# bdaiinstitute/vlfm

Measured on NVIDIA H100. Metric: value-map steps/sec (ITM+cone-fuse), higher is better.
Workload: dtype f16

## Files before the change

### vlfm_b200/csrc/gemm_wgmma.cu

```cuda
#include <cuda.h>
#include <cuda_fp16.h>
#include <math.h>
#include <stdlib.h>

#include "common.cuh"

namespace vlfm {

constexpr int BM = 128;
constexpr int BK = 64;
constexpr int GEMM_THREADS = 384;
constexpr int GEMM_CONSUMERS = 256;

__device__ __forceinline__ void mbar_expect_tx(uint32_t bar, uint32_t bytes) {
  asm volatile("mbarrier.arrive.expect_tx.shared::cta.b64 _, [%0], %1;" ::"r"(bar), "r"(bytes) : "memory");
}
__device__ __forceinline__ void mbar_arrive(uint32_t bar) {
  asm volatile("mbarrier.arrive.shared::cta.b64 _, [%0];" ::"r"(bar) : "memory");
}
__device__ __forceinline__ void tma_load_2d(uint32_t dst, const CUtensorMap* map, int x, int y, uint32_t bar) {
  asm volatile(
      "cp.async.bulk.tensor.2d.shared::cluster.global.mbarrier::complete_tx::bytes [%0], [%1, {%3, %4}], [%2];"
      ::"r"(dst), "l"(map), "r"(bar), "r"(x), "r"(y) : "memory");
}
__device__ __forceinline__ uint64_t wgmma_desc_k128(uint32_t saddr) {
  return (uint64_t)((saddr & 0x3FFFF) >> 4) | ((uint64_t)1 << 16) | ((uint64_t)(1024 >> 4) << 32) | ((uint64_t)1 << 62);
}
__device__ __forceinline__ void wg_fence() { asm volatile("wgmma.fence.sync.aligned;" ::: "memory"); }
__device__ __forceinline__ void wg_commit() { asm volatile("wgmma.commit_group.sync.aligned;" ::: "memory"); }
template <int PENDING>
__device__ __forceinline__ void wg_wait() { asm volatile("wgmma.wait_group.sync.aligned %0;" ::"n"(PENDING) : "memory"); }

#define VLFM_D4(d, i) "+f"(d[i]), "+f"(d[i + 1]), "+f"(d[i + 2]), "+f"(d[i + 3])
#define VLFM_D16(d, i) VLFM_D4(d, i), VLFM_D4(d, i + 4), VLFM_D4(d, i + 8), VLFM_D4(d, i + 12)
template <int BN> struct Wgmma;
template <> struct Wgmma<32> {
  static __device__ __forceinline__ void mma(float (&d)[16], uint64_t a, uint64_t b, uint32_t acc) {
    asm volatile(
        "{\n\t.reg .pred p;\n\tsetp.ne.b32 p, %18, 0;\n\t"
        "wgmma.mma_async.sync.aligned.m64n32k16.f32.f16.f16 "
        "{%0,%1,%2,%3,%4,%5,%6,%7,%8,%9,%10,%11,%12,%13,%14,%15}, %16, %17, p, 1, 1, 0, 0;\n\t}"
        : VLFM_D16(d, 0) : "l"(a), "l"(b), "r"(acc));
  }
};
template <> struct Wgmma<64> {
  static __device__ __forceinline__ void mma(float (&d)[32], uint64_t a, uint64_t b, uint32_t acc) {
    asm volatile(
        "{\n\t.reg .pred p;\n\tsetp.ne.b32 p, %34, 0;\n\t"
        "wgmma.mma_async.sync.aligned.m64n64k16.f32.f16.f16 "
        "{%0,%1,%2,%3,%4,%5,%6,%7,%8,%9,%10,%11,%12,%13,%14,%15,"
        "%16,%17,%18,%19,%20,%21,%22,%23,%24,%25,%26,%27,%28,%29,%30,%31}, %32, %33, p, 1, 1, 0, 0;\n\t}"
        : VLFM_D16(d, 0), VLFM_D16(d, 16) : "l"(a), "l"(b), "r"(acc));
  }
};
template <> struct Wgmma<96> {
  static __device__ __forceinline__ void mma(float (&d)[48], uint64_t a, uint64_t b, uint32_t acc) {
    asm volatile(
        "{\n\t.reg .pred p;\n\tsetp.ne.b32 p, %50, 0;\n\t"
        "wgmma.mma_async.sync.aligned.m64n96k16.f32.f16.f16 "
        "{%0,%1,%2,%3,%4,%5,%6,%7,%8,%9,%10,%11,%12,%13,%14,%15,"
        "%16,%17,%18,%19,%20,%21,%22,%23,%24,%25,%26,%27,%28,%29,%30,%31,"
        "%32,%33,%34,%35,%36,%37,%38,%39,%40,%41,%42,%43,%44,%45,%46,%47}, %48, %49, p, 1, 1, 0, 0;\n\t}"
        : VLFM_D16(d, 0), VLFM_D16(d, 16), VLFM_D16(d, 32) : "l"(a), "l"(b), "r"(acc));
  }
};
template <> struct Wgmma<128> {
  static __device__ __forceinline__ void mma(float (&d)[64], uint64_t a, uint64_t b, uint32_t acc) {
    asm volatile(
        "{\n\t.reg .pred p;\n\tsetp.ne.b32 p, %66, 0;\n\t"
        "wgmma.mma_async.sync.aligned.m64n128k16.f32.f16.f16 "
        "{%0,%1,%2,%3,%4,%5,%6,%7,%8,%9,%10,%11,%12,%13,%14,%15,"
        "%16,%17,%18,%19,%20,%21,%22,%23,%24,%25,%26,%27,%28,%29,%30,%31,"
        "%32,%33,%34,%35,%36,%37,%38,%39,%40,%41,%42,%43,%44,%45,%46,%47,"
        "%48,%49,%50,%51,%52,%53,%54,%55,%56,%57,%58,%59,%60,%61,%62,%63}, %64, %65, p, 1, 1, 0, 0;\n\t}"
        : VLFM_D16(d, 0), VLFM_D16(d, 16), VLFM_D16(d, 32), VLFM_D16(d, 48) : "l"(a), "l"(b), "r"(acc));
  }
};
#undef VLFM_D16
#undef VLFM_D4

struct GemmArgs {
  const float* bias;
  void* out;
  int M, N, K, ldo, epi;
  int kb_per_split;
  long long split_stride;
// ... 375 lines not shown
      const uint32_t a0 = smem_u32(sA + s * A_BYTES) + (uint32_t)wg * (64 * BK * 2), b0 = smem_u32(sB + s * B_BYTES);
      wg_fence();
#pragma unroll
      for (int k = 0; k < BK / 16; ++k)
        Wgmma<BN>::mma(acc, wgmma_desc_k128(a0 + k * 32), wgmma_desc_k128(b0 + k * 32), (kb > kb_lo || k > 0) ? 1u : 0u);
      wg_commit();
      if (f < BN) {
        const uint8_t* wrow = sB + (size_t)s * B_BYTES + (size_t)f * 128;
        const int k0 = (kb - kb_lo) * BK + hk * 32;
        float a[GEMM_TAIL_MAX];
#pragma unroll
        for (int r = 0; r < GEMM_TAIL_MAX; ++r) a[r] = 0.f;
#pragma unroll
        for (int c = 0; c < 4; ++c) {
          const uint4 wv = *reinterpret_cast<const uint4*>(wrow + (((hk * 4 + c) ^ (f & 7)) << 4));
          const __half2* wh = reinterpret_cast<const __half2*>(&wv);
#pragma unroll
          for (int r = 0; r < GEMM_TAIL_MAX; ++r) {
            if (r < g.tail_rows) {
              const uint4 xv = *reinterpret_cast<const uint4*>(sx + (size_t)r * kslice + k0 + c * 8);
              const __half2* xh = reinterpret_cast<const __half2*>(&xv);
#pragma unroll
              for (int e = 0; e < 4; ++e) {
                const float2 xf = __half22float2(xh[e]), wf = __half22float2(wh[e]);
                a[r] = fmaf(xf.x, wf.x, a[r]); a[r] = fmaf(xf.y, wf.y, a[r]);
              }
            }
          }
        }
#pragma unroll
        for (int r = 0; r < GEMM_TAIL_MAX; ++r) tacc[r] += a[r];
      }
      wg_wait<1>();
      if (kb > kb_lo) {
        __syncwarp();
        if (lane == 0) mbar_arrive(empty0 + 8 * (s == 0 ? STAGES - 1 : s - 1));
      }
      if (++s == STAGES) { s = 0; ph ^= 1; }
    }
    wg_wait<0>();
#pragma unroll
    for (int r = 0; r < GEMM_TAIL_MAX; ++r) tacc[r] += __shfl_xor_sync(0xffffffffu, tacc[r], 1);
    if (s_cl == 1) {
      if (hk == 0 && f < BN && n_blk * BN + f < g.N) {
#pragma unroll
        for (int r = 0; r < GEMM_TAIL_MAX; ++r)
          if (r < g.tail_rows) epilogue_store2(g, CS_BM + r, n_blk * BN + f, tacc[r] + sbias[f], 0.f, false, false);
      }
      epilogue_frag<BN>(acc, wg * 64 + wq * 16, n_blk, g, false, true, sbias);
    } else {
      asm volatile("bar.sync 1, 512;" ::: "memory");
      const int r_up = wg * 64 + wq * 16 + (lane >> 2), cq = (lane & 3) * 2;
#pragma unroll
      for (int j = 0; j < BN / 8; ++j) {
        *reinterpret_cast<float2*>(part + r_up * LDP + j * 8 + cq) = make_float2(acc[4 * j], acc[4 * j + 1]);
        *reinterpret_cast<float2*>(part + (r_up + 8) * LDP + j * 8 + cq) = make_float2(acc[4 * j + 2], acc[4 * j + 3]);
      }
      if (hk == 0 && f < BN) {
#pragma unroll
        for (int r = 0; r < GEMM_TAIL_MAX; ++r)
          if (r < g.tail_rows) part[(CS_BM + r) * LDP + f] = tacc[r];
      }
    }
  }
  if (s_cl > 1) {
    cluster_sync_all();
    if (warp >= 4) {
      const int et = threadIdx.x - (CS_THREADS - CS_CONSUMERS);
      const int rows = CS_BM + g.tail_rows, r0 = rank * rows / s_cl, r1 = (rank + 1) * rows / s_cl;
      const uint32_t base = smem_u32(part);
      for (int i = et; i < (r1 - r0) * (BN / 2); i += CS_CONSUMERS) {
        const int row = r0 + i / (BN / 2), c = (i % (BN / 2)) * 2, n = n_blk * BN + c;
        if (n >= g.N) continue;
        const uint32_t off = base + (uint32_t)(row * LDP + c) * 4;
        float2 sum = ld_peer_f2(off, 0);
        for (int p = 1; p < s_cl; ++p) { const float2 v = ld_peer_f2(off, p); sum.x += v.x; sum.y += v.y; }
        epilogue_store2(g, row, n, sum.x + sbias[c], sum.y + sbias[c + 1], n + 1 < g.N, false);
      }
    }
    cluster_sync_all();
  }
}

template <int BN, int STAGES>
__global__ void __launch_bounds__(GEMM_THREADS, 1)
gemm_f16x2_wgmma_kernel(const __grid_constant__ CUtensorMap tmA, const __grid_constant__ CUtensorMap tmAl,
                        const __grid_constant__ CUtensorMap tmB, const __grid_constant__ CUtensorMap tmBl, GemmArgs g) {
  constexpr uint32_t A_BYTES = BM * BK * 2, B_BYTES = BN * BK * 2;

  extern __shared__ uint8_t smem_raw[];
  uint8_t* sA = smem_align_1024(smem_raw);
  uint8_t* sAl = sA + STAGES * A_BYTES;
  uint8_t* sB = sAl + STAGES * A_BYTES;
  uint8_t* sBl = sB + STAGES * B_BYTES;
  uint64_t* bars = reinterpret_cast<uint64_t*>(sBl + STAGES * B_BYTES);
  const uint32_t full0 = smem_u32(bars), empty0 = smem_u32(bars + STAGES);
  float* sbias = reinterpret_cast<float*>(bars + 2 * STAGES);

  pdl_trigger();
  const int warp = threadIdx.x >> 5, lane = threadIdx.x & 31;
  const int n_blk = blockIdx.x, m_blk = blockIdx.y;
  const int kb_begin = blockIdx.z * g.kb_per_split;
  const int num_k = min((g.K + BK - 1) / BK - kb_begin, g.kb_per_split);
  const bool split = gridDim.z > 1;

  if (warp == 0 && lane == 0) {
    asm volatile("prefetch.tensormap [%0];" ::"l"(&tmA) : "memory");
    asm volatile("prefetch.tensormap [%0];" ::"l"(&tmAl) : "memory");
    asm volatile("prefetch.tensormap [%0];" ::"l"(&tmB) : "memory");
    asm volatile("prefetch.tensormap [%0];" ::"l"(&tmBl) : "memory");
    for (int i = 0; i < STAGES; ++i) { mbar_init(full0 + 8 * i, 1); mbar_init(empty0 + 8 * i, GEMM_CONSUMERS / 32); }
    asm volatile("fence.mbarrier_init.release.cluster;" ::: "memory");
    asm volatile("fence.proxy.async.shared::cta;" ::: "memory");
  }
  __syncthreads();

  if (warp == 0) {
    if (lane == 0) {
      const int pre = num_k < STAGES ? num_k : STAGES;
      const uint32_t a_tx = (uint32_t)g.a_box_rows * BK * 2;
      for (int kb = 0; kb < pre; ++kb) {
        mbar_expect_tx(full0 + 8 * kb, 2 * (a_tx + B_BYTES));
        tma_load_2d(smem_u32(sB + kb * B_BYTES), &tmB, (kb_begin + kb) * BK, n_blk * BN, full0 + 8 * kb);
        tma_load_2d(smem_u32(sBl + kb * B_BYTES), &tmBl, (kb_begin + kb) * BK, n_blk * BN, full0 + 8 * kb);
      }
      pdl_wait();
      for (int kb = 0; kb < pre; ++kb) {
        tma_load_2d(smem_u32(sA + kb * A_BYTES), &tmA, (kb_begin + kb) * BK, m_blk * BM, full0 + 8 * kb);
        tma_load_2d(smem_u32(sAl + kb * A_BYTES), &tmAl, (kb_begin + kb) * BK, m_blk * BM, full0 + 8 * kb);
      }
      int s = pre == STAGES ? 0 : pre; uint32_t ph = pre == STAGES ? 1 : 0;
      for (int kb = pre; kb < num_k; ++kb) {
        mbar_wait(empty0 + 8 * s, ph ^ 1);
        mbar_expect_tx(full0 + 8 * s, 2 * (a_tx + B_BYTES));
        tma_load_2d(smem_u32(sA + s * A_BYTES), &tmA, (kb_begin + kb) * BK, m_blk * BM, full0 + 8 * s);
        tma_load_2d(smem_u32(sAl + s * A_BYTES), &tmAl, (kb_begin + kb) * BK, m_blk * BM, full0 + 8 * s);
        tma_load_2d(smem_u32(sB + s * B_BYTES), &tmB, (kb_begin + kb) * BK, n_blk * BN, full0 + 8 * s);
        tma_load_2d(smem_u32(sBl + s * B_BYTES), &tmBl, (kb_begin + kb) * BK, n_blk * BN, full0 + 8 * s);
        if (++s == STAGES) { s = 0; ph ^= 1; }
      }
    }
  } else if (warp >= 4) {
    const int wg = (warp >> 2) - 1, wq = warp & 3;
    const int et = threadIdx.x - (GEMM_THREADS - GEMM_CONSUMERS);
    const int wg_row0 = m_blk * BM + wg * 64;
    const bool active = wg_row0 < g.M;
    if (et < BN) { const int n = n_blk * BN + et; sbias[et] = (g.bias && n < g.N) ? __ldg(g.bias + n) : 0.f; }
    asm volatile("bar.sync 1, 256;" ::: "memory");
    pdl_wait();
    if (!active) {
      int s = 0; uint32_t ph = 0;
      for (int kb = 0; kb < num_k; ++kb) {
        mbar_wait(full0 + 8 * s, ph);
        __syncwarp();
        if (lane == 0) mbar_arrive(empty0 + 8 * s);
        if (++s == STAGES) { s = 0; ph ^= 1; }
      }
      return;
    }
    float acc[BN / 2], corr[BN / 2];
#pragma unroll
    for (int i = 0; i < BN / 2; ++i) { acc[i] = 0.f; corr[i] = 0.f; }
    int s = 0; uint32_t ph = 0;
    for (int kb = 0; kb < num_k; ++kb) {
      mbar_wait(full0 + 8 * s, ph);
      const uint32_t wg_off = (uint32_t)wg * (64 * BK * 2);
      const uint32_t a0 = smem_u32(sA + s * A_BYTES) + wg_off, al0 = smem_u32(sAl + s * A_BYTES) + wg_off;
      const uint32_t b0 = smem_u32(sB + s * B_BYTES), bl0 = smem_u32(sBl + s * B_BYTES);
      wg_fence();
#pragma unroll
      for (int k = 0; k < BK / 16; ++k) {
        const uint64_t da = wgmma_desc_k128(a0 + k * 32), dal = wgmma_desc_k128(al0 + k * 32);
        const uint64_t db = wgmma_desc_k128(b0 + k * 32), dbl = wgmma_desc_k128(bl0 + k * 32);
        const uint32_t first = (kb > 0 || k > 0) ? 1u : 0u;
        Wgmma<BN>::mma(acc, da, db, first);
        Wgmma<BN>::mma(corr, dal, db, first);
        Wgmma<BN>::mma(corr, da, dbl, 1u);
      }
      wg_commit();
      wg_wait<1>();
      if (kb > 0) {
        __syncwarp();
        if (lane == 0) mbar_arrive(empty0 + 8 * (s == 0 ? STAGES - 1 : s - 1));
      }
      if (++s == STAGES) { s = 0; ph ^= 1; }
    }
    wg_wait<0>();
#pragma unroll
    for (int i = 0; i < BN / 2; ++i) acc[i] = fmaf(corr[i], 1.f / X2_SCALE, acc[i]);
    epilogue_frag<BN>(acc, wg_row0 + wq * 16, n_blk, g, split, blockIdx.z == 0, sbias);
  }
}

typedef CUresult (*EncodeTiledFn)(CUtensorMap*, CUtensorMapDataType, cuuint32_t, void*, const cuuint64_t*,
                                  const cuuint64_t*, const cuuint32_t*, const cuuint32_t*, CUtensorMapInterleave,
                                  CUtensorMapSwizzle, CUtensorMapL2promotion, CUtensorMapFloatOOBfill);

static EncodeTiledFn get_encode() {
  static EncodeTiledFn fn = nullptr;
  static bool tried = false;
  if (!tried) {
    tried = true;
    void* p = nullptr;
    cudaDriverEntryPointQueryResult q;
    if (cudaGetDriverEntryPoint("cuTensorMapEncodeTiled", &p, cudaEnableDefault, &q) == cudaSuccess &&
        q == cudaDriverEntryPointSuccess)
      fn = reinterpret_cast<EncodeTiledFn>(p);
  }
  return fn;
}

static int make_map(CUtensorMap* m, const void* base, int rows, int cols, int ld, int boxRows) {
  EncodeTiledFn enc = get_encode();
  if (!enc) { set_error("cuTensorMapEncodeTiled entry point unavailable"); return VLFM_E_DRIVER; }
  cuuint64_t dims[2] = {(cuuint64_t)cols, (cuuint64_t)rows};
  cuuint64_t strides[1] = {(cuuint64_t)ld * 2};
  cuuint32_t box[2] = {(cuuint32_t)BK, (cuuint32_t)boxRows};
  cuuint32_t estr[2] = {1, 1};
  CUresult r = enc(m, CU_TENSOR_MAP_DATA_TYPE_FLOAT16, 2, const_cast<void*>(base), dims, strides, box, estr,
                   CU_TENSOR_MAP_INTERLEAVE_NONE, CU_TENSOR_MAP_SWIZZLE_128B, CU_TENSOR_MAP_L2_PROMOTION_L2_256B,
                   CU_TENSOR_MAP_FLOAT_OOB_FILL_NONE);
  if (r != CUDA_SUCCESS) { set_error("cuTensorMapEncodeTiled failed (%d) rows=%d cols=%d ld=%d", (int)r, rows, cols, ld); return VLFM_E_DRIVER; }
  return VLFM_OK;
}

template <int BN, int STAGES, bool SILU = false>
static int launch_gemm(const CUtensorMap& ta, const void* W, int ldw, const GemmArgs& g, cudaStream_t st) {
  if constexpr (!SILU) {
    if (g.epi == VLFM_EPI_BIAS_SILU_F16) return launch_gemm<BN, STAGES, true>(ta, W, ldw, g, st);
  }
  CUtensorMap tb;
  int rc = make_map(&tb, W, g.N, g.K, ldw, BN);
  if (rc) return rc;
  constexpr size_t smem = (size_t)STAGES * (BM * BK * 2 + BN * BK * 2) + 2 * STAGES * 8 + 1024 + BN * 4 +
                          (size_t)GEMM_TAIL_MAX * GEMM_TAIL_KMAX * 2;
  static_assert(smem <= 227 * 1024, "GEMM stage ring exceeds the 227 KB a block may use");
  static bool configured = false;
  if (!configured) {
    rc = check_cuda(cudaFuncSetAttribute(gemm_f16_wgmma_kernel<BN, STAGES, SILU>, cudaFuncAttributeMaxDynamicSharedMemorySize, (int)smem), "cudaFuncSetAttribute(gemm)");
    if (rc) return rc;
    configured = true;
  }
  const int num_k = (g.K + BK - 1) / BK;
  dim3 grid((g.N + BN - 1) / BN, g.tail_rows > 0 ? g.M / BM : (g.M + BM - 1) / BM, (num_k + g.kb_per_split - 1) / g.kb_per_split);
  if (g.sk.ctas > 0) grid = dim3(g.sk.ctas);
  rc = check_cuda(launch_pdl(gemm_f16_wgmma_kernel<BN, STAGES, SILU>, grid, dim3(GEMM_THREADS), smem, st, ta, tb, g), "gemm_f16_wgmma_kernel");
  if (rc) return rc;
  count_launch();
  return VLFM_OK;
}


template <int BN, int STAGES>
static int launch_gemm_x2(const CUtensorMap& ta, const CUtensorMap& tal, const void* W, const void* Wl, int ldw, const GemmArgs& g, cudaStream_t st) {
  CUtensorMap tb, tbl;
  int rc = make_map(&tb, W, g.N, g.K, ldw, BN);
  if (!rc) rc = make_map(&tbl, Wl, g.N, g.K, ldw, BN);
  if (rc) return rc;
  constexpr size_t smem = (size_t)STAGES * 2 * (BM * BK * 2 + BN * BK * 2) + 2 * STAGES * 8 + 1024 + BN * 4;
  static_assert(smem <= 227 * 1024, "x2 GEMM stage ring exceeds the 227 KB a block may use");
  static bool configured = false;
  if (!configured) {
    rc = check_cuda(cudaFuncSetAttribute(gemm_f16x2_wgmma_kernel<BN, STAGES>, cudaFuncAttributeMaxDynamicSharedMemorySize, (int)smem), "cudaFuncSetAttribute(gemm x2)");
    if (rc) return rc;
    configured = true;
  }
  const int num_k = (g.K + BK - 1) / BK;
  dim3 grid((g.N + BN - 1) / BN, (g.M + BM - 1) / BM, (num_k + g.kb_per_split - 1) / g.kb_per_split);
  rc = check_cuda(launch_pdl(gemm_f16x2_wgmma_kernel<BN, STAGES>, grid, dim3(GEMM_THREADS), smem, st, ta, tal, tb, tbl, g), "gemm_f16x2_wgmma_kernel");
  if (rc) return rc;
  count_launch();
  return VLFM_OK;
}

template <int BN, int STAGES>
struct Csplit {
  static constexpr size_t smem = (size_t)STAGES * (CS_BM * BK * 2 + BN * BK * 2) + 2 * STAGES * 8 + 1024 + BN * 4 +
                                 (size_t)GEMM_TAIL_MAX * GEMM_TAIL_KMAX * 2;
  static_assert(smem <= 227 * 1024, "cluster-split GEMM stage ring exceeds the 227 KB a block may use");
  static int configure() {
    static int rc = -1;
    if (rc < 0) rc = check_cuda(cudaFuncSetAttribute(gemm_f16_csplit_wgmma_kernel<BN, STAGES>, cudaFuncAttributeMaxDynamicSharedMemorySize, (int)smem),
                                "cudaFuncSetAttribute(gemm csplit)");
    return rc;
  }
  static int max_clusters(int s) {
    static int fit[9] = {-1, -1, -1, -1, -1, -1, -1, -1, -1};
    if (fit[s] < 0) {
      fit[s] = 0;
      if (configure()) return 0;
      cudaLaunchConfig_t cfg{};
      cfg.gridDim = dim3(s); cfg.blockDim = dim3(CS_THREADS); cfg.dynamicSmemBytes = smem;
      cudaLaunchAttribute attr[1];
      attr[0].id = cudaLaunchAttributeClusterDimension;
      attr[0].val.clusterDim.x = s; attr[0].val.clusterDim.y = 1; attr[0].val.clusterDim.z = 1;
      cfg.attrs = attr; cfg.numAttrs = 1;
      int n = 0;
      if (cudaOccupancyMaxActiveClusters(&n, gemm_f16_csplit_wgmma_kernel<BN, STAGES>, &cfg) == cudaSuccess) fit[s] = n;
      else cudaGetLastError();
    }
    return fit[s];
  }
  static int launch(const CUtensorMap& ta, const void* W, int ldw, const GemmArgs& g, int s, cudaStream_t st) {
    CUtensorMap tb;
    int rc = make_map(&tb, W, g.N, g.K, ldw, BN);
    if (!rc) rc = configure();
    if (rc) return rc;
    cudaLaunchConfig_t cfg{};
    cfg.gridDim = dim3(((g.N + BN - 1) / BN) * s); cfg.blockDim = dim3(CS_THREADS); cfg.dynamicSmemBytes = smem; cfg.stream = st;
    cudaLaunchAttribute attr[2];
    attr[0].id = cudaLaunchAttributeClusterDimension;
    attr[0].val.clusterDim.x = s; attr[0].val.clusterDim.y = 1; attr[0].val.clusterDim.z = 1;
    attr[1].id = cudaLaunchAttributeProgrammaticStreamSerialization;
    attr[1].val.programmaticStreamSerializationAllowed = 1;
    cfg.attrs = attr; cfg.numAttrs = pdl_enabled() ? 2 : 1;
    rc = check_cuda(cudaLaunchKernelEx(&cfg, gemm_f16_csplit_wgmma_kernel<BN, STAGES>, ta, tb, g), "gemm_f16_csplit_wgmma_kernel");
    if (rc) return rc;
    count_launch();
    return VLFM_OK;
  }
};

}

using namespace vlfm;

static int gemm_dispatch(const void* d_A, const void* d_W, int M, int N, int K, int lda, int ldw, GemmArgs g, void* stream, float* d_partials,
                         size_t partial_bytes, SplitK* layout, bool csplit);

static int sm_count() {
  static int sms = 0;
  if (!sms) { int dev = 0; cudaGetDevice(&dev); if (cudaDeviceGetAttribute(&sms, cudaDevAttrMultiProcessorCount, dev) != cudaSuccess || sms < 1) sms = 132; }
  return sms;
}

extern "C" int vlfm_gemm_f16(const void* d_A, const void* d_W, const float* d_bias, void* d_out, int M, int N,
                             int K, int lda, int ldw, int ldo, int epilogue, void* stream) {
  if (!d_A || !d_W || !d_out || M < 1 || N < 1 || K < 1) { set_error("vlfm_gemm_f16: bad argument"); return VLFM_E_INVALID; }
  if ((K & 7) || (lda & 7) || (ldw & 7) || (ldo & 7) || ((uintptr_t)d_A & 15) || ((uintptr_t)d_W & 15) || ((uintptr_t)d_out & 15)) {
    set_error("vlfm_gemm_f16: K, lda, ldw, ldo must be multiples of 8 and pointers 16-byte aligned"); return VLFM_E_INVALID; }
  const bool csplit = (epilogue & VLFM_EPI_CLUSTER_SPLIT) != 0 && (epilogue & ~VLFM_EPI_CLUSTER_SPLIT) != VLFM_EPI_BIAS_SILU_F16;
  epilogue &= ~VLFM_EPI_CLUSTER_SPLIT;
  if (epilogue < 0 || (epilogue > 4 && epilogue != VLFM_EPI_BIAS_SILU_F16)) { set_error("vlfm_gemm_f16: unknown epilogue %d", epilogue); return VLFM_E_INVALID; }
  GemmArgs g{d_bias, d_out, M, N, K, ldo, epilogue, (K + BK - 1) / BK, 0, nullptr, 0, 0, 0, nullptr, BM};
  return gemm_dispatch(d_A, d_W, M, N, K, lda, ldw, g, stream, nullptr, 0, nullptr, csplit);
}

constexpr double CS_RED_FIXED_BYTES = 16384;
constexpr long long CS_MIN_WEIGHTS = 8ll << 20;
static bool csplit_eligible(int M, int N, int K) {
  const char* e = getenv("VLFM_GEMM_CSPLIT");
  const int mode = (e && e[0]) ? atoi(e) : 1;
// ... 84 lines not shown
      return launch_gemm<128, 6>(ta, d_W, ldw, g, st);
    }
  }
  if (tiles128 <= sms && !resid) {
    const int bns[4] = {128, 96, 64, 32};
    long long best = -1;
    for (int bn : bns) {
      const long long tl = (long long)rt * ((N + bn - 1) / bn), cols = (tl + sms - 1) / sms * bn;
      if (best < 0 || cols < best) { best = cols; best_bn = bn; }
    }
  } else {
    double best_t = 1e30;
    const int bns[3] = {128, 64, 32};
    for (int tm = 0; tm < (tail ? 2 : 1); ++tm) {
      const bool use_tail = tail && tm == 0;
      const int mte = use_tail ? M / BM : mt;
      for (int bi = 0; bi < 3; ++bi) {
        const int bn = bns[bi], nt = (N + bn - 1) / bn;
        int smax = resid && !(d_partials && tiles128 < sms) ? num_k / 4 : 1;
        if (smax < 1) smax = 1;
        if (smax > 8) smax = 8;
        if (smax > split_cap) smax = (int)split_cap;
        for (int sp = 1; sp <= smax; ++sp) {
          const double ctas = (double)mte * nt * sp;
          const int kb = (num_k + sp - 1) / sp;
          const double waves = (double)(long)((ctas + sms - 1) / sms);
          const double active = ctas < sms ? ctas : sms;
          const double kb_kbytes = (double)(128 + bn) * 128 / 1024.0;
          double per_kb = active * kb_kbytes / 5500.0;
          if (per_kb < 0.33) per_kb = 0.33;
          double c0 = bn == 128 ? 3.8 + 0.22 * sp : (bn == 64 ? 3.0 : 2.6) + (sp > 1 ? 0.1 * sp : 0.0);
          if (use_tail) c0 += bn == 128 ? 0.9 : 0.3;
          const double t = waves * (c0 + kb * per_kb);
          if (t < best_t) { best_t = t; best_bn = bn; best_s = sp; best_tail = use_tail; }
        }
      }
    }
  }
  if (force) {
    int fb = 0, fs = 0;
    if (sscanf(force, "%d:%d", &fb, &fs) == 2 && (fb == 128 || fb == 96 || fb == 64 || fb == 32) && fs >= 1) {
      best_bn = fb;
      best_s = resid ? (fs > num_k ? num_k : fs) : 1;
      if (best_s > split_cap) best_s = (int)split_cap;
    }
  }
  g.kb_per_split = (num_k + best_s - 1) / best_s;
  if (best_tail) { g.a_tail = (const __half*)d_A + (size_t)(M / BM) * BM * lda; g.lda = lda; g.tail_rows = rem; g.tail_row0 = (M / BM) * BM; }
  const int launched_splits = (num_k + g.kb_per_split - 1) / g.kb_per_split;
  if (d_partials && launched_splits > 1 && resid && (size_t)launched_splits * (size_t)M * (size_t)N * 4 <= partial_bytes) {
    g.epi = VLFM_EPI_PARTIAL_F32; g.out = d_partials; g.ldo = N; g.split_stride = (long long)M * N;
    if (layout) *layout = SplitK{launched_splits, (long long)M * N};
  }
  if (best_bn == 128) return launch_gemm<128, 6>(ta, d_W, ldw, g, st);
  if (best_bn == 96) return launch_gemm<96, 7>(ta, d_W, ldw, g, st);
  if (best_bn == 64) return launch_gemm<64, 8>(ta, d_W, ldw, g, st);
  return launch_gemm<32, 8>(ta, d_W, ldw, g, st);
}

extern "C" int vlfm_layernorm(const float* d_x, const float* d_gamma, const float* d_beta, void* d_out16, float* d_out32,
                   int rows, int D, int ldx, int ldo16, int ldo32, float eps, void* stream);
namespace vlfm {
int layernorm_reduce_impl(float* d_x, const float* d_partials, const SplitK& sk, const float* d_gamma, const float* d_beta, void* d_out16,
                          void* d_out16_lo, float* d_out32, int rows, int D, int ldx, int ldo16, int ldo32, float eps, void* stream);
}

extern "C" int vlfm_gemm_f16_resid_ln(const void* d_A, const void* d_W, const float* d_bias, float* d_x, int M, int N, int K,
                                      int lda, int ldw, int ldx, const float* d_gamma, const float* d_beta, void* d_out16,
                                      int ld16, float* d_out32, int ld32, float eps, float* d_partials, size_t partial_bytes, void* stream) {
  if (!d_A || !d_W || !d_x || !d_gamma || !d_beta || (!d_out16 && !d_out32) || M < 1 || N < 1 || K < 1) {
    set_error("vlfm_gemm_f16_resid_ln: bad argument"); return VLFM_E_INVALID; }
  if ((K & 7) || (lda & 7) || (ldw & 7) || (ldx & 7) || (N & 3) || (ld16 & 3) || (ld32 & 3) || ((uintptr_t)d_A & 15) || ((uintptr_t)d_W & 15) ||
      ((uintptr_t)d_x & 15) || ((uintptr_t)d_partials & 15)) { set_error("vlfm_gemm_f16_resid_ln: alignment (K, strides %% 8; N %% 4; 16-byte pointers)"); return VLFM_E_INVALID; }
  int rc = layernorm_check("vlfm_gemm_f16_resid_ln", d_x, d_gamma, d_beta, d_out16, nullptr, d_out32, N, ldx, ld16, ld32);
  if (rc) return rc;
  GemmArgs g{d_bias, d_x, M, N, K, ldx, VLFM_EPI_BIAS_RESID_F32, (K + BK - 1) / BK, 0, nullptr, 0, 0, 0, nullptr, BM};
  SplitK layout;
  rc = gemm_dispatch(d_A, d_W, M, N, K, lda, ldw, g, stream, d_partials, partial_bytes, &layout, d_partials != nullptr);
  if (rc) return rc;
  if (layout.splits != 1) return layernorm_reduce_impl(d_x, d_partials, layout, d_gamma, d_beta, d_out16, nullptr, d_out32, M, N, ldx, ld16, ld32, eps, stream);
  return vlfm_layernorm(d_x, d_gamma, d_beta, d_out16, d_out32, M, N, ldx, ld16, ld32, eps, stream);
}

static int gemm_x2_dispatch(const void* d_A_hi, const void* d_A_lo, const void* d_W_hi, const void* d_W_lo, int M, int N, int K, int lda, int ldw,
                            GemmArgs g, void* stream, float* d_partials, size_t partial_bytes, int* splits_out) {
  if (splits_out) *splits_out = 1;
  const int rem = M % BM;
  if (M > BM && rem >= 1 && rem <= 32 && (g.epi == VLFM_EPI_BIAS_F32 || g.epi == VLFM_EPI_BIAS_GELU_F16X2)) {
    const int m0 = M - rem;
    GemmArgs g0 = g; g0.M = m0;
    int rc0 = gemm_x2_dispatch(d_A_hi, d_A_lo, d_W_hi, d_W_lo, m0, N, K, lda, ldw, g0, stream, nullptr, 0, nullptr);
    if (rc0) return rc0;
    GemmArgs g1 = g; g1.M = rem;
    const size_t esz = g.epi == VLFM_EPI_BIAS_F32 ? 4 : 2;
    g1.out = (uint8_t*)g.out + (size_t)m0 * g.ldo * esz;
    if (g.out_lo) g1.out_lo = (uint8_t*)g.out_lo + (size_t)m0 * g.ldo * 2;
    return gemm_x2_dispatch((const __half*)d_A_hi + (size_t)m0 * lda, (const __half*)d_A_lo + (size_t)m0 * lda, d_W_hi, d_W_lo, rem, N, K, lda, ldw, g1,
                            stream, nullptr, 0, nullptr);
  }
  CUtensorMap ta, tal;
  g.a_box_rows = M <= 32 ? 32 : (M <= 64 ? 64 : BM);
  int rc = make_map(&ta, d_A_hi, M, K, lda, g.a_box_rows);
  if (!rc) rc = make_map(&tal, d_A_lo, M, K, lda, g.a_box_rows);
  if (rc) return rc;
  const int mt = (M + BM - 1) / BM, num_k = (K + BK - 1) / BK;
  int bn = 32;
  if (mt >= 2 && N >= 4096) bn = 128;
  else if ((long)mt * ((N + 63) / 64) >= 96) bn = 64;
  const int tiles = mt * ((N + bn - 1) / bn);
  int sp = 1;
  if (g.epi == VLFM_EPI_BIAS_RESID_F32 && d_partials) {
    sp = sm_count() / tiles; if (sp > num_k / 3) sp = num_k / 3; if (sp > 8) sp = 8; if (sp < 1) sp = 1;
  }
  g.kb_per_split = (num_k + sp - 1) / sp;
  const int launched = (num_k + g.kb_per_split - 1) / g.kb_per_split;
  if (launched > 1) {
    if ((size_t)launched * (size_t)M * (size_t)N * 4 > partial_bytes) { g.kb_per_split = num_k; }
    else { g.epi = VLFM_EPI_PARTIAL_F32; g.out = d_partials; g.ldo = N; g.split_stride = (long long)M * N; if (splits_out) *splits_out = launched; }
  }
  cudaStream_t st = (cudaStream_t)stream;
  if (bn == 128) return launch_gemm_x2<128, 3>(ta, tal, d_W_hi, d_W_lo, ldw, g, st);
  if (bn == 64) return launch_gemm_x2<64, 4>(ta, tal, d_W_hi, d_W_lo, ldw, g, st);
  return launch_gemm_x2<32, 5>(ta, tal, d_W_hi, d_W_lo, ldw, g, st);
}

static int x2_args_ok(const char* who, const void* a, const void* al, const void* w, const void* wl, const void* out, int M, int N, int K, int lda, int ldw, int ldo) {
  if (!a || !al || !w || !wl || !out || M < 1 || N < 1 || K < 1) { set_error("%s: bad argument", who); return VLFM_E_INVALID; }
  if ((K & 7) || (lda & 7) || (ldw & 7) || (ldo & 7) || ((uintptr_t)a & 15) || ((uintptr_t)al & 15) || ((uintptr_t)w & 15) || ((uintptr_t)wl & 15) || ((uintptr_t)out & 15)) {
    set_error("%s: K, lda, ldw, ldo must be multiples of 8 and pointers 16-byte aligned", who); return VLFM_E_INVALID; }
  return VLFM_OK;
}

extern "C" int vlfm_gemm_f16x2(const void* d_A_hi, const void* d_A_lo, const void* d_W_hi, const void* d_W_lo, const float* d_bias, void* d_out,
                               void* d_out_lo, int M, int N, int K, int lda, int ldw, int ldo, int epilogue, void* stream) {
  int rc = x2_args_ok("vlfm_gemm_f16x2", d_A_hi, d_A_lo, d_W_hi, d_W_lo, d_out, M, N, K, lda, ldw, ldo);
  if (rc) return rc;
  if (epilogue != VLFM_EPI_BIAS_F32 && epilogue != VLFM_EPI_BIAS_RESID_F32 && epilogue != VLFM_EPI_BIAS_GELU_F16X2) {
    set_error("vlfm_gemm_f16x2: epilogue %d unsupported (fp32, fp32 residual, GELU x2)", epilogue); return VLFM_E_INVALID; }
  if (epilogue == VLFM_EPI_BIAS_GELU_F16X2 && (!d_out_lo || ((uintptr_t)d_out_lo & 15))) { set_error("vlfm_gemm_f16x2: d_out_lo missing / unaligned"); return VLFM_E_INVALID; }
  GemmArgs g{d_bias, d_out, M, N, K, ldo, epilogue, (K + BK - 1) / BK, 0, nullptr, 0, 0, 0, d_out_lo, BM};
  return gemm_x2_dispatch(d_A_hi, d_A_lo, d_W_hi, d_W_lo, M, N, K, lda, ldw, g, stream, nullptr, 0, nullptr);
}

extern "C" int vlfm_layernorm_x2(const float* d_x, const float* d_gamma, const float* d_beta, void* d_out_hi, void* d_out_lo, float* d_out32,
                                 int rows, int D, int ldx, int ldo16, int ldo32, float eps, void* stream);
extern "C" int vlfm_layernorm_reduce_x2(float* d_x, const float* d_partials, int splits, long long split_stride, const float* d_gamma,
                                        const float* d_beta, void* d_out_hi, void* d_out_lo, float* d_out32, int rows, int D, int ldx, int ldo16,
                                        int ldo32, float eps, void* stream);

extern "C" int vlfm_gemm_f16x2_resid_ln(const void* d_A_hi, const void* d_A_lo, const void* d_W_hi, const void* d_W_lo, const float* d_bias,
                                        float* d_x, int M, int N, int K, int lda, int ldw, int ldx, const float* d_gamma, const float* d_beta,
                                        void* d_out_hi, void* d_out_lo, int ld16, float* d_out32, int ld32, float eps, float* d_partials,
                                        size_t partial_bytes, void* stream) {
  int rc = x2_args_ok("vlfm_gemm_f16x2_resid_ln", d_A_hi, d_A_lo, d_W_hi, d_W_lo, d_x, M, N, K, lda, ldw, ldx);
  if (rc) return rc;
  if (!d_gamma || !d_beta || !d_out_hi || !d_out_lo || (N & 3) || (ld16 & 3) || (ld32 & 3) || ((uintptr_t)d_partials & 15)) {
    set_error("vlfm_gemm_f16x2_resid_ln: bad argument / alignment"); return VLFM_E_INVALID; }
  rc = layernorm_check("vlfm_gemm_f16x2_resid_ln", d_x, d_gamma, d_beta, d_out_hi, d_out_lo, d_out32, N, ldx, ld16, ld32);
  if (rc) return rc;
  GemmArgs g{d_bias, d_x, M, N, K, ldx, VLFM_EPI_BIAS_RESID_F32, (K + BK - 1) / BK, 0, nullptr, 0, 0, 0, nullptr, BM};
  int splits = 1;
  rc = gemm_x2_dispatch(d_A_hi, d_A_lo, d_W_hi, d_W_lo, M, N, K, lda, ldw, g, stream, d_partials, partial_bytes, &splits);
  if (rc) return rc;
  if (splits > 1) return vlfm_layernorm_reduce_x2(d_x, d_partials, splits, (long long)M * N, d_gamma, d_beta, d_out_hi, d_out_lo, d_out32, M, N, ldx, ld16, ld32, eps, stream);
  return vlfm_layernorm_x2(d_x, d_gamma, d_beta, d_out_hi, d_out_lo, d_out32, M, N, ldx, ld16, ld32, eps, stream);
}
```

Measured before the change: 234.6.

## Size x2 GEMM stage ring to A box rows and fuse remainder into paired launch

Reorganizes the split-precision wgmma GEMM smem ring into interleaved per-stage slots sized to the actual TMA A-box rows. This allows many more pipeline stages, up to twelve, and fewer consumer warps when M is small. It also merges the main-tile GEMM and the small M-remainder GEMM into one paired kernel launch, removing a second launch and its tail serialization. The trade-offs are more template instantiations, larger shared memory per block, and a legacy env switch; the paired kernel launches 384 threads even for the remainder CTAs.

Result: no change. 236.8, median of 6 (+0.9%).

```diff
diff --git a/vlfm_b200/csrc/gemm_wgmma.cu b/vlfm_b200/csrc/gemm_wgmma.cu
--- a/vlfm_b200/csrc/gemm_wgmma.cu
+++ b/vlfm_b200/csrc/gemm_wgmma.cu
@@ -2,6 +2,7 @@
 #include <cuda_fp16.h>
 #include <math.h>
 #include <stdlib.h>
+#include <string.h>
 
 #include "common.cuh"
 
@@ -543,24 +544,39 @@
   }
 }
 
-template <int BN, int STAGES>
-__global__ void __launch_bounds__(GEMM_THREADS, 1)
-gemm_f16x2_wgmma_kernel(const __grid_constant__ CUtensorMap tmA, const __grid_constant__ CUtensorMap tmAl,
-                        const __grid_constant__ CUtensorMap tmB, const __grid_constant__ CUtensorMap tmBl, GemmArgs g) {
-  constexpr uint32_t A_BYTES = BM * BK * 2, B_BYTES = BN * BK * 2;
+constexpr int X2_MAX_STAGES = 12;
+template <int BN, int AROWS>
+struct X2Ring {
+  static constexpr uint32_t A_BYTES = AROWS * BK * 2, B_BYTES = BN * BK * 2;
+  static constexpr uint32_t STAGE_BYTES = 2 * (A_BYTES + B_BYTES);
+  static constexpr int CONSUMERS = AROWS > 64 ? 256 : 128;
+  static constexpr int THREADS = 128 + CONSUMERS;
+  static constexpr int FIT = (int)((227 * 1024 - 1024 - BN * 4) / (STAGE_BYTES + 16));
+  static constexpr int STAGES = FIT < X2_MAX_STAGES ? FIT : X2_MAX_STAGES;
+  static constexpr size_t smem = (size_t)STAGES * (STAGE_BYTES + 16) + 1024 + BN * 4;
+  static_assert(AROWS == 32 || AROWS == 64 || AROWS == BM, "A stage rows: the TMA box rows");
+  static_assert(smem <= 227 * 1024, "x2 GEMM stage ring exceeds the 227 KB a block may use");
+};
+
+template <int BN, int AROWS>
+__device__ __forceinline__ void gemm_x2_cta(const CUtensorMap& tmA, const CUtensorMap& tmAl, const CUtensorMap& tmB, const CUtensorMap& tmBl,
+                                            const GemmArgs& g, int n_blk, int m_blk) {
+  using R = X2Ring<BN, AROWS>;
+  constexpr int STAGES = R::STAGES, CONSUMERS = R::CONSUMERS;
+  constexpr uint32_t A_BYTES = R::A_BYTES, B_BYTES = R::B_BYTES, STAGE_BYTES = R::STAGE_BYTES;
 
   extern __shared__ uint8_t smem_raw[];
-  uint8_t* sA = smem_align_1024(smem_raw);
-  uint8_t* sAl = sA + STAGES * A_BYTES;
-  uint8_t* sB = sAl + STAGES * A_BYTES;
-  uint8_t* sBl = sB + STAGES * B_BYTES;
-  uint64_t* bars = reinterpret_cast<uint64_t*>(sBl + STAGES * B_BYTES);
+  uint8_t* ring = smem_align_1024(smem_raw);
+  auto sA = [&](int s) { return smem_u32(ring + s * STAGE_BYTES); };
+  auto sAl = [&](int s) { return smem_u32(ring + s * STAGE_BYTES + A_BYTES); };
+  auto sB = [&](int s) { return smem_u32(ring + s * STAGE_BYTES + 2 * A_BYTES); };
+  auto sBl = [&](int s) { return smem_u32(ring + s * STAGE_BYTES + 2 * A_BYTES + B_BYTES); };
+  uint64_t* bars = reinterpret_cast<uint64_t*>(ring + STAGES * STAGE_BYTES);
   const uint32_t full0 = smem_u32(bars), empty0 = smem_u32(bars + STAGES);
   float* sbias = reinterpret_cast<float*>(bars + 2 * STAGES);
 
   pdl_trigger();
   const int warp = threadIdx.x >> 5, lane = threadIdx.x & 31;
-  const int n_blk = blockIdx.x, m_blk = blockIdx.y;
   const int kb_begin = blockIdx.z * g.kb_per_split;
   const int num_k = min((g.K + BK - 1) / BK - kb_begin, g.kb_per_split);
   const bool split = gridDim.z > 1;
@@ -570,7 +586,7 @@
     asm volatile("prefetch.tensormap [%0];" ::"l"(&tmAl) : "memory");
     asm volatile("prefetch.tensormap [%0];" ::"l"(&tmB) : "memory");
     asm volatile("prefetch.tensormap [%0];" ::"l"(&tmBl) : "memory");
-    for (int i = 0; i < STAGES; ++i) { mbar_init(full0 + 8 * i, 1); mbar_init(empty0 + 8 * i, GEMM_CONSUMERS / 32); }
+    for (int i = 0; i < STAGES; ++i) { mbar_init(full0 + 8 * i, 1); mbar_init(empty0 + 8 * i, CONSUMERS / 32); }
     asm volatile("fence.mbarrier_init.release.cluster;" ::: "memory");
     asm volatile("fence.proxy.async.shared::cta;" ::: "memory");
   }
@@ -582,32 +598,32 @@
       const uint32_t a_tx = (uint32_t)g.a_box_rows * BK * 2;
       for (int kb = 0; kb < pre; ++kb) {
         mbar_expect_tx(full0 + 8 * kb, 2 * (a_tx + B_BYTES));
-        tma_load_2d(smem_u32(sB + kb * B_BYTES), &tmB, (kb_begin + kb) * BK, n_blk * BN, full0 + 8 * kb);
-        tma_load_2d(smem_u32(sBl + kb * B_BYTES), &tmBl, (kb_begin + kb) * BK, n_blk * BN, full0 + 8 * kb);
+        tma_load_2d(sB(kb), &tmB, (kb_begin + kb) * BK, n_blk * BN, full0 + 8 * kb);
+        tma_load_2d(sBl(kb), &tmBl, (kb_begin + kb) * BK, n_blk * BN, full0 + 8 * kb);
       }
       pdl_wait();
       for (int kb = 0; kb < pre; ++kb) {
-        tma_load_2d(smem_u32(sA + kb * A_BYTES), &tmA, (kb_begin + kb) * BK, m_blk * BM, full0 + 8 * kb);
-        tma_load_2d(smem_u32(sAl + kb * A_BYTES), &tmAl, (kb_begin + kb) * BK, m_blk * BM, full0 + 8 * kb);
+        tma_load_2d(sA(kb), &tmA, (kb_begin + kb) * BK, m_blk * BM, full0 + 8 * kb);
+        tma_load_2d(sAl(kb), &tmAl, (kb_begin + kb) * BK, m_blk * BM, full0 + 8 * kb);
       }
       int s = pre == STAGES ? 0 : pre; uint32_t ph = pre == STAGES ? 1 : 0;
       for (int kb = pre; kb < num_k; ++kb) {
         mbar_wait(empty0 + 8 * s, ph ^ 1);
         mbar_expect_tx(full0 + 8 * s, 2 * (a_tx + B_BYTES));
-        tma_load_2d(smem_u32(sA + s * A_BYTES), &tmA, (kb_begin + kb) * BK, m_blk * BM, full0 + 8 * s);
-        tma_load_2d(smem_u32(sAl + s * A_BYTES), &tmAl, (kb_begin + kb) * BK, m_blk * BM, full0 + 8 * s);
-        tma_load_2d(smem_u32(sB + s * B_BYTES), &tmB, (kb_begin + kb) * BK, n_blk * BN, full0 + 8 * s);
-        tma_load_2d(smem_u32(sBl + s * B_BYTES), &tmBl, (kb_begin + kb) * BK, n_blk * BN, full0 + 8 * s);
+        tma_load_2d(sA(s), &tmA, (kb_begin + kb) * BK, m_blk * BM, full0 + 8 * s);
+        tma_load_2d(sAl(s), &tmAl, (kb_begin + kb) * BK, m_blk * BM, full0 + 8 * s);
+        tma_load_2d(sB(s), &tmB, (kb_begin + kb) * BK, n_blk * BN, full0 + 8 * s);
+        tma_load_2d(sBl(s), &tmBl, (kb_begin + kb) * BK, n_blk * BN, full0 + 8 * s);
         if (++s == STAGES) { s = 0; ph ^= 1; }
       }
     }
-  } else if (warp >= 4) {
-    const int wg = (warp >> 2) - 1, wq = warp & 3;
-    const int et = threadIdx.x - (GEMM_THREADS - GEMM_CONSUMERS);
+  } else if (warp >= 4 && warp < 4 + CONSUMERS / 32) {
+    const int wg = CONSUMERS > 128 ? (warp >> 2) - 1 : 0, wq = warp & 3;
+    const int et = threadIdx.x - 128;
     const int wg_row0 = m_blk * BM + wg * 64;
     const bool active = wg_row0 < g.M;
     if (et < BN) { const int n = n_blk * BN + et; sbias[et] = (g.bias && n < g.N) ? __ldg(g.bias + n) : 0.f; }
-    asm volatile("bar.sync 1, 256;" ::: "memory");
+    asm volatile("bar.sync 1, %0;" ::"n"(CONSUMERS) : "memory");
     pdl_wait();
     if (!active) {
       int s = 0; uint32_t ph = 0;
@@ -626,8 +642,8 @@
     for (int kb = 0; kb < num_k; ++kb) {
       mbar_wait(full0 + 8 * s, ph);
       const uint32_t wg_off = (uint32_t)wg * (64 * BK * 2);
-      const uint32_t a0 = smem_u32(sA + s * A_BYTES) + wg_off, al0 = smem_u32(sAl + s * A_BYTES) + wg_off;
-      const uint32_t b0 = smem_u32(sB + s * B_BYTES), bl0 = smem_u32(sBl + s * B_BYTES);
+      const uint32_t a0 = sA(s) + wg_off, al0 = sAl(s) + wg_off;
+      const uint32_t b0 = sB(s), bl0 = sBl(s);
       wg_fence();
 #pragma unroll
       for (int k = 0; k < BK / 16; ++k) {
@@ -651,6 +667,25 @@
     for (int i = 0; i < BN / 2; ++i) acc[i] = fmaf(corr[i], 1.f / X2_SCALE, acc[i]);
     epilogue_frag<BN>(acc, wg_row0 + wq * 16, n_blk, g, split, blockIdx.z == 0, sbias);
   }
+}
+
+template <int BN, int AROWS>
+__global__ void __launch_bounds__(X2Ring<BN, AROWS>::THREADS, 1)
+gemm_f16x2_wgmma_kernel(const __grid_constant__ CUtensorMap tmA, const __grid_constant__ CUtensorMap tmAl,
+                        const __grid_constant__ CUtensorMap tmB, const __grid_constant__ CUtensorMap tmBl, GemmArgs g) {
+  gemm_x2_cta<BN, AROWS>(tmA, tmAl, tmB, tmBl, g, blockIdx.x, blockIdx.y);
+}
+
+template <int BN0, int BN1>
+__global__ void __launch_bounds__(X2Ring<BN0, BM>::THREADS, 1)
+gemm_f16x2_pair_kernel(const __grid_constant__ CUtensorMap tmA, const __grid_constant__ CUtensorMap tmAl,
+                       const __grid_constant__ CUtensorMap tmB, const __grid_constant__ CUtensorMap tmBl, const __grid_constant__ CUtensorMap tmA1,
+                       const __grid_constant__ CUtensorMap tmAl1, const __grid_constant__ CUtensorMap tmB1, const __grid_constant__ CUtensorMap tmBl1,
+                       GemmArgs g, GemmArgs g1, int ctas0) {
+  static_assert(X2Ring<BN1, 32>::THREADS <= X2Ring<BN0, BM>::THREADS, "remainder CTA fits the block");
+  const int t = blockIdx.x, nt0 = (g.N + BN0 - 1) / BN0;
+  if (t < ctas0) gemm_x2_cta<BN0, BM>(tmA, tmAl, tmB, tmBl, g, t % nt0, t / nt0);
+  else gemm_x2_cta<BN1, 32>(tmA1, tmAl1, tmB1, tmBl1, g1, t - ctas0, 0);
 }
 
 typedef CUresult (*EncodeTiledFn)(CUtensorMap*, CUtensorMapDataType, cuuint32_t, void*, const cuuint64_t*,
@@ -712,23 +747,46 @@
 }
 
 
-template <int BN, int STAGES>
+template <int BN, int AROWS>
 static int launch_gemm_x2(const CUtensorMap& ta, const CUtensorMap& tal, const void* W, const void* Wl, int ldw, const GemmArgs& g, cudaStream_t st) {
+  using R = X2Ring<BN, AROWS>;
   CUtensorMap tb, tbl;
   int rc = make_map(&tb, W, g.N, g.K, ldw, BN);
   if (!rc) rc = make_map(&tbl, Wl, g.N, g.K, ldw, BN);
   if (rc) return rc;
-  constexpr size_t smem = (size_t)STAGES * 2 * (BM * BK * 2 + BN * BK * 2) + 2 * STAGES * 8 + 1024 + BN * 4;
-  static_assert(smem <= 227 * 1024, "x2 GEMM stage ring exceeds the 227 KB a block may use");
   static bool configured = false;
   if (!configured) {
-    rc = check_cuda(cudaFuncSetAttribute(gemm_f16x2_wgmma_kernel<BN, STAGES>, cudaFuncAttributeMaxDynamicSharedMemorySize, (int)smem), "cudaFuncSetAttribute(gemm x2)");
+    rc = check_cuda(cudaFuncSetAttribute(gemm_f16x2_wgmma_kernel<BN, AROWS>, cudaFuncAttributeMaxDynamicSharedMemorySize, (int)R::smem), "cudaFuncSetAttribute(gemm x2)");
     if (rc) return rc;
     configured = true;
   }
   const int num_k = (g.K + BK - 1) / BK;
   dim3 grid((g.N + BN - 1) / BN, (g.M + BM - 1) / BM, (num_k + g.kb_per_split - 1) / g.kb_per_split);
-  rc = check_cuda(launch_pdl(gemm_f16x2_wgmma_kernel<BN, STAGES>, grid, dim3(GEMM_THREADS), smem, st, ta, tal, tb, tbl, g), "gemm_f16x2_wgmma_kernel");
+  rc = check_cuda(launch_pdl(gemm_f16x2_wgmma_kernel<BN, AROWS>, grid, dim3(R::THREADS), R::smem, st, ta, tal, tb, tbl, g), "gemm_f16x2_wgmma_kernel");
+  if (rc) return rc;
+  count_launch();
+  return VLFM_OK;
+}
+
+template <int BN0, int BN1>
+static int launch_gemm_x2_pair(const CUtensorMap& ta, const CUtensorMap& tal, const CUtensorMap& ta1, const CUtensorMap& tal1, const void* W,
+                               const void* Wl, int ldw, const GemmArgs& g, const GemmArgs& g1, cudaStream_t st) {
+  CUtensorMap tb, tbl, tb1, tbl1;
+  int rc = make_map(&tb, W, g.N, g.K, ldw, BN0);
+  if (!rc) rc = make_map(&tbl, Wl, g.N, g.K, ldw, BN0);
+  if (!rc) rc = make_map(&tb1, W, g.N, g.K, ldw, BN1);
+  if (!rc) rc = make_map(&tbl1, Wl, g.N, g.K, ldw, BN1);
+  if (rc) return rc;
+  constexpr size_t smem = X2Ring<BN0, BM>::smem > X2Ring<BN1, 32>::smem ? X2Ring<BN0, BM>::smem : X2Ring<BN1, 32>::smem;
+  static bool configured = false;
+  if (!configured) {
+    rc = check_cuda(cudaFuncSetAttribute(gemm_f16x2_pair_kernel<BN0, BN1>, cudaFuncAttributeMaxDynamicSharedMemorySize, (int)smem), "cudaFuncSetAttribute(gemm x2 pair)");
+    if (rc) return rc;
+    configured = true;
+  }
+  const int ctas0 = ((g.N + BN0 - 1) / BN0) * (g.M / BM), ctas1 = (g.N + BN1 - 1) / BN1;
+  rc = check_cuda(launch_pdl(gemm_f16x2_pair_kernel<BN0, BN1>, dim3(ctas0 + ctas1), dim3(X2Ring<BN0, BM>::THREADS), smem, st, ta, tal, tb, tbl,
+                             ta1, tal1, tb1, tbl1, g, g1, ctas0), "gemm_f16x2_pair_kernel");
   if (rc) return rc;
   count_launch();
   return VLFM_OK;
@@ -979,6 +1037,10 @@
   return vlfm_layernorm(d_x, d_gamma, d_beta, d_out16, d_out32, M, N, ldx, ld16, ld32, eps, stream);
 }
 
+static bool x2_ring_legacy() {
+  const char* e = getenv("VLFM_X2_RING");
+  return e && !strcmp(e, "legacy");
+}
 static int gemm_x2_dispatch(const void* d_A_hi, const void* d_A_lo, const void* d_W_hi, const void* d_W_lo, int M, int N, int K, int lda, int ldw,
                             GemmArgs g, void* stream, float* d_partials, size_t partial_bytes, int* splits_out) {
   if (splits_out) *splits_out = 1;
@@ -986,14 +1048,25 @@
   if (M > BM && rem >= 1 && rem <= 32 && (g.epi == VLFM_EPI_BIAS_F32 || g.epi == VLFM_EPI_BIAS_GELU_F16X2)) {
     const int m0 = M - rem;
     GemmArgs g0 = g; g0.M = m0;
-    int rc0 = gemm_x2_dispatch(d_A_hi, d_A_lo, d_W_hi, d_W_lo, m0, N, K, lda, ldw, g0, stream, nullptr, 0, nullptr);
-    if (rc0) return rc0;
     GemmArgs g1 = g; g1.M = rem;
     const size_t esz = g.epi == VLFM_EPI_BIAS_F32 ? 4 : 2;
     g1.out = (uint8_t*)g.out + (size_t)m0 * g.ldo * esz;
     if (g.out_lo) g1.out_lo = (uint8_t*)g.out_lo + (size_t)m0 * g.ldo * 2;
-    return gemm_x2_dispatch((const __half*)d_A_hi + (size_t)m0 * lda, (const __half*)d_A_lo + (size_t)m0 * lda, d_W_hi, d_W_lo, rem, N, K, lda, ldw, g1,
-                            stream, nullptr, 0, nullptr);
+    const __half* a1 = (const __half*)d_A_hi + (size_t)m0 * lda;
+    const __half* al1 = (const __half*)d_A_lo + (size_t)m0 * lda;
+    if (!x2_ring_legacy() && m0 >= 2 * BM && N >= 4096 && (N + 63) / 64 >= 96) {
+      CUtensorMap ta, tal, ta1, tal1;
+      g0.a_box_rows = BM; g1.a_box_rows = 32;
+      int rc = make_map(&ta, d_A_hi, m0, K, lda, BM);
+      if (!rc) rc = make_map(&tal, d_A_lo, m0, K, lda, BM);
+      if (!rc) rc = make_map(&ta1, a1, rem, K, lda, 32);
+      if (!rc) rc = make_map(&tal1, al1, rem, K, lda, 32);
+      if (rc) return rc;
+      return launch_gemm_x2_pair<128, 64>(ta, tal, ta1, tal1, d_W_hi, d_W_lo, ldw, g0, g1, (cudaStream_t)stream);
+    }
+    int rc0 = gemm_x2_dispatch(d_A_hi, d_A_lo, d_W_hi, d_W_lo, m0, N, K, lda, ldw, g0, stream, nullptr, 0, nullptr);
+    if (rc0) return rc0;
+    return gemm_x2_dispatch(a1, al1, d_W_hi, d_W_lo, rem, N, K, lda, ldw, g1, stream, nullptr, 0, nullptr);
   }
   CUtensorMap ta, tal;
   g.a_box_rows = M <= 32 ? 32 : (M <= 64 ? 64 : BM);
@@ -1016,9 +1089,16 @@
     else { g.epi = VLFM_EPI_PARTIAL_F32; g.out = d_partials; g.ldo = N; g.split_stride = (long long)M * N; if (splits_out) *splits_out = launched; }
   }
   cudaStream_t st = (cudaStream_t)stream;
-  if (bn == 128) return launch_gemm_x2<128, 3>(ta, tal, d_W_hi, d_W_lo, ldw, g, st);
-  if (bn == 64) return launch_gemm_x2<64, 4>(ta, tal, d_W_hi, d_W_lo, ldw, g, st);
-  return launch_gemm_x2<32, 5>(ta, tal, d_W_hi, d_W_lo, ldw, g, st);
+  const int arows = x2_ring_legacy() ? BM : g.a_box_rows;
+  if (bn == 128) return launch_gemm_x2<128, BM>(ta, tal, d_W_hi, d_W_lo, ldw, g, st);
+  if (bn == 64) {
+    if (arows == 32) return launch_gemm_x2<64, 32>(ta, tal, d_W_hi, d_W_lo, ldw, g, st);
+    if (arows == 64) return launch_gemm_x2<64, 64>(ta, tal, d_W_hi, d_W_lo, ldw, g, st);
+    return launch_gemm_x2<64, BM>(ta, tal, d_W_hi, d_W_lo, ldw, g, st);
+  }
+  if (arows == 32) return launch_gemm_x2<32, 32>(ta, tal, d_W_hi, d_W_lo, ldw, g, st);
+  if (arows == 64) return launch_gemm_x2<32, 64>(ta, tal, d_W_hi, d_W_lo, ldw, g, st);
+  return launch_gemm_x2<32, BM>(ta, tal, d_W_hi, d_W_lo, ldw, g, st);
 }
 
 static int x2_args_ok(const char* who, const void* a, const void* al, const void* w, const void* wl, const void* out, int M, int N, int K, int lda, int ldw, int ldo) {
```
